# varunagrawal/tiny-faces-pytorch

Measured on AMD Instinct MI355X. Metric: train img/s @ 500x500 bs=12/GPU, higher is better.
Workload: dtype bf16; 1 GPU; configs[2]: bs=12/GPU synthetic 500x500 crops + random boxes; dense_overlap targets on GPU, ResNet-101 hybrid-head fwd, criterion, bwd, fused SGD; global_batch=12, image=500x500, templates=25, parallelism=dp1, weights=random init (tamed kaiming), fp32 master + bf16 MFMA operands

## Files before the change

### tiny-faces-pytorch_amd/csrc/capi.hip

```cpp
#include "common.h"
#include "debug_api.h"

static const char* const kSymbols[] = {
    "tf_version", "tf_build_id", "tf_symbol_count", "tf_symbol_name",
    "tf_targets_workspace_bytes", "tf_dense_overlap_targets", "tf_dense_overlap_iou", "tf_pairwise_iou_distance",
    "tf_nms_workspace_bytes", "tf_nms_f64", "tf_nms_batched_workspace_bytes", "tf_nms_f64_batched",
    "tf_decode_workspace_bytes", "tf_decode_compact",
    "tf_criterion_workspace_bytes", "tf_criterion_fwd_bwd",
    "tf_sgd_step", "tf_image_prepare",
    "tf_conv_mtiles", "tf_conv2d", "tf_pack_weight", "tf_pack_weights_batched", "tf_pack_weights_tiled", "tf_conv2d_wgrad", "tf_conv2d_wgrad_group", "tf_wgrad_workspace_bytes", "tf_unpack_dw",
    "tf_stem_im2col", "tf_stem_conv", "tf_stem_wgrad", "tf_maxpool_fwd", "tf_maxpool_bwd", "tf_maxpool_bwd_stats", "tf_colstats_blocks", "tf_colstats",
    "tf_bn_finalize", "tf_bn_fold", "tf_bn_bwd_finalize", "tf_bn_bwd_apply", "tf_bn_relu", "tf_bn_add_relu",
    "tf_bn_relu_fused", "tf_bn_add_relu_fused", "tf_bn_bwd_apply_fused",
#if TF_EXP
    "tf_conv2d_bnbwd", "tf_conv2d_bnfwd",
#endif
    "tf_upsample_add_crop", "tf_upsample_add_crop_bwd", "tf_reduce_partials",
    "tf_detnet_num_params", "tf_detnet_param_name", "tf_detnet_param_numel", "tf_detnet_workspace_bytes",
    "tf_detnet_out_shape", "tf_detnet_param_region_bytes", "tf_detnet_forward", "tf_detnet_backward", "tf_detnet_ctx_create", "tf_detnet_ctx_destroy", "tf_detnet_forward_ctx", "tf_detnet_backward_ctx", "tf_comm_available", "tf_comm_unique_id", "tf_comm_init", "tf_comm_destroy", "tf_comm_rank", "tf_comm_world", "tf_allreduce_bucket", "tf_comm_join", "tf_comm_allreduce_hook",
    "tf_detnet_set_dual_stream", "tf_detnet_set_grad_events", "tf_detnet_set_grad_callback",
    "tf_detnet_trunk_num_params", "tf_detnet_trunk_param_name", "tf_detnet_trunk_param_numel", "tf_detnet_trunk_workspace_bytes",
    "tf_detnet_trunk_param_region_bytes", "tf_detnet_trunk_forward_ctx", "tf_detnet_trunk_backward_ctx",
    "tf_set_stat_rows", "tf_get_stat_rows", "tf_profile_enable", "tf_profile_collect", "tf_profile_shapes",
};

namespace tf {
static thread_local hipEvent_t g_next_stop_event = nullptr;
void set_next_stop_event(hipEvent_t e) { g_next_stop_event = e; }
hipEvent_t take_next_stop_event() { hipEvent_t e = g_next_stop_event; g_next_stop_event = nullptr; return e; }
}

extern "C" int tf_version(void) { return 610; }
#ifndef TF_BUILD_ID
#define TF_BUILD_ID "unstamped"
#endif
extern "C" const char* tf_build_id(void) { return TF_EXP ? TF_BUILD_ID "+x" : TF_BUILD_ID; }
static int g_stat_rows = 8;
extern "C" int tf_set_stat_rows(int rows) { g_stat_rows = rows <= 0 ? (1 << 30) : (rows > TF_STAT_ROWS ? TF_STAT_ROWS : rows); return TF_OK; }
extern "C" int tf_get_stat_rows(void) { return g_stat_rows; }
extern "C" int tf_symbol_count(void) { return (int)(sizeof(kSymbols) / sizeof(kSymbols[0])); }
extern "C" const char* tf_symbol_name(int i) { return (i >= 0 && i < tf_symbol_count()) ? kSymbols[i] : nullptr; }

namespace {
typedef __bf16 bf16x4 __attribute__((ext_vector_type(4)));
__global__ void probe_tr16_kernel(unsigned short* out) {
  __shared__ __attribute__((aligned(16))) unsigned short lds[256];
  for (int i = threadIdx.x; i < 256; i += 64) lds[i] = (unsigned short)i;
  __syncthreads();
  typedef __attribute__((address_space(3))) bf16x4 lds_bf16x4;
  const bf16x4 v = __builtin_amdgcn_ds_read_tr16_b64_v4bf16((lds_bf16x4*)(lds + threadIdx.x * 4));
  const uint2 raw = __builtin_bit_cast(uint2, v);
  out[threadIdx.x * 4 + 0] = (unsigned short)(raw.x & 0xffff); out[threadIdx.x * 4 + 1] = (unsigned short)(raw.x >> 16);
  out[threadIdx.x * 4 + 2] = (unsigned short)(raw.y & 0xffff); out[threadIdx.x * 4 + 3] = (unsigned short)(raw.y >> 16);
}
}
extern "C" int tf_probe_tr16(unsigned short* out256, void* stream) {
  hipLaunchKernelGGL(probe_tr16_kernel, dim3(1), dim3(64), 0, (hipStream_t)stream, out256);
  TF_CHECK_LAUNCH();
  return TF_OK;
}
```

### tiny-faces-pytorch_amd/csrc/detnet.hip

```cpp
#include <cstdio>
#include <cstdlib>
#include <cstring>
#include <string>
#include <utility>
#include <vector>

#include "common.h"
#include "tuning.h"

extern "C" {
int tf_stem_im2col(const float*, int, int, int, int, void*, int, void*);
int tf_stem_conv(int, const float*, int, int, int, const void*, int, void*, int, const float*, const float*, float*, int*, void*);
int tf_stem_wgrad(int, const float*, int, int, int, const void*, const void*, const float*, const float*, const float*, float*, void*);
int tf_maxpool_fwd(int, const void*, int, int, int, int, const float*, const float*, void*, uint8_t*, void*);
int tf_maxpool_bwd(int, const void*, const uint8_t*, const void*, const float*, const float*, int, int, int, int, void*, void*);
int tf_maxpool_bwd_stats(int, const void*, const uint8_t*, const void*, const float*, const float*, int, int, int, int, void*, float*, int*, void*);
int tf_colstats_blocks(int, int, int);
int tf_colstats(int, const void*, const void*, const void*, const void*, int, int, int, float*, void*);
int tf_bn_finalize(const float*, int, int, int, float, const float*, const float*, float, float, float*, float*, float*, float*, float*,
                   float*, int, void*);
int tf_bn_fold(const float*, const float*, const float*, const float*, float, int, float*, float*, void*);
int tf_bn_bwd_finalize(const float*, int, int, int, int, int, float, const float*, const float*, const float*, float*, float*, float*, float*,
                       float*, int, void*);
int tf_bn_bwd_apply(int, const void*, const void*, const void*, const float*, const float*, const float*, int64_t, int, void*, void*);
// ... 683 lines not shown
extern "C" int tf_detnet_forward(int dtype, int training, const float* x, int N, int H, int W, int nout, void* const* params, float eps,
                                 float mom, float* out, void* ws, size_t ws_bytes, int flags, void* stream_) {
  return tf_detnet_forward_ctx(nullptr, g_force_single ? 1 : 0, dtype, training, x, N, H, W, nout, params, eps, mom, out, ws, ws_bytes, flags, stream_);
}

namespace {

void bn_backward_coefs(Ctx& c, const ConvUnit& u, int C, BnBuf& b, const float* partial, int nblk, int nk, int kidx, int ld, float count,
                       int clear = 1) {
  c.chk(tf_bn_bwd_finalize(partial, nblk, nk, kidx, ld, C, count, c.P(u.gamma), b.mean, b.invstd, c.G(u.gamma), c.G(u.beta), b.cA, b.cB,
                           b.cD, clear, c.stream));
}

tf_wgrad_args wgrad_args(const Ctx& c, const ConvUnit& u, int cout, int N, int H, int W, int OH, int OW, const void* x, int ldx, const void* dy,
                         int lddy, int cin_override = 0, int k_override = 0, int dw_ld = 0) {
  tf_wgrad_args w;
  memset(&w, 0, sizeof(w));
  const int cin = cin_override ? cin_override : u.cin, k = k_override ? k_override : u.k;
  w.dtype = c.dtype; w.N = N; w.H = H; w.W = W; w.Cin = cin; w.OH = OH; w.OW = OW; w.Cout = cout; w.KH = k; w.KW = k;
  w.stride = u.stride; w.pad = u.pad; w.ldx = ldx; w.lddy = lddy; w.x = x; w.dy = dy; w.dw_oihw = c.G(u.w);
  w.dw_ld = dw_ld ? dw_ld : cin * k * k;
  return w;
}

void wgrad(Ctx& c, const ConvUnit& u, int cout, int N, int H, int W, int OH, int OW, const void* x, int ldx, const void* dy, int lddy,
           const BnBuf* pro, int cin_override = 0, int k_override = 0, int dw_ld = 0, float* packed_scratch = nullptr, size_t scratch_floats = 0) {
  const bool skip = tf::tuning().dbg_skip_wgrad;
  if (skip) return;
  const int cin = cin_override ? cin_override : u.cin, k = k_override ? k_override : u.k;
  tf_wgrad_args w = wgrad_args(c, u, cout, N, H, W, OH, OW, x, ldx, dy, lddy, cin_override, k_override, dw_ld);
  if (pro) { w.pro_scale = pro->scale; w.pro_shift = pro->shift; w.pro_relu = 1; }
  if (k > 1 && packed_scratch && c.grads_zeroed) {
    w.partial_ws = packed_scratch; w.partial_ws_bytes = scratch_floats * 4;
    if (tf_wgrad_workspace_bytes(&w) != 0 && tf_wgrad_workspace_bytes(&w) <= w.partial_ws_bytes) {
      const bool w3_off = tf::tuning().wgrad3_off;
      if (!w3_off) { c.chk(tf_conv2d_wgrad(&w, c.wstream())); return; }
    }
    w.partial_ws = nullptr; w.partial_ws_bytes = 0;
  }
  if (k > 1 && packed_scratch) {
    float* oihw = w.dw_oihw;
    w.dw_oihw = packed_scratch; w.packed = 1;
    if (hipMemsetAsync(packed_scratch, 0, (size_t)cout * w.dw_ld * 4, c.wstream()) != hipSuccess) c.chk(TF_ERR_LAUNCH);
    c.chk(tf_conv2d_wgrad(&w, c.wstream()));
    c.chk(tf_unpack_dw(packed_scratch, cout, cin, k * k, oihw, c.wstream()));
    return;
  }
  if (!c.grads_zeroed && hipMemsetAsync(w.dw_oihw, 0, (size_t)cout * w.dw_ld * 4, c.wstream()) != hipSuccess) c.chk(TF_ERR_LAUNCH);
  c.chk(tf_conv2d_wgrad(&w, c.wstream()));
}

}

static std::vector<std::pair<int, hipEvent_t>> g_grad_events;
extern "C" int tf_detnet_set_grad_events(const int* blocks, void* const* events, int n) {
  g_grad_events.clear();
  if (n < 0 || (n > 0 && (!blocks || !events))) return TF_ERR_ARG;
  for (int k = 0; k < n; ++k) g_grad_events.emplace_back(blocks[k], (hipEvent_t)events[k]);
  return TF_OK;
}
static tf_grad_ready_fn g_grad_cb = nullptr;
static void* g_grad_cb_user = nullptr;
extern "C" int tf_detnet_set_grad_callback(tf_grad_ready_fn fn, void* user) { g_grad_cb = fn; g_grad_cb_user = user; return TF_OK; }
static void record_grad_events(const tf_detnet_hooks* h, int block, hipStream_t s, int& rc) {
  if (!h) return;
  bool registered = false;
  for (int k = 0; k < h->n; ++k)
    if (h->blocks[k] == block) {
      registered = true;
      hipEvent_t e = h->events ? (hipEvent_t)h->events[k] : nullptr;
      if (e && hipEventRecord(e, s) != hipSuccess && rc == TF_OK) rc = TF_ERR_LAUNCH;
// ... 325 lines not shown
```

### tiny-faces-pytorch_amd/csrc/wgrad.hip

```cpp
#include "common.h"
#include "tuning.h"
#include "profile.h"

int tf_wgrad_dma_launch(const tf_wgrad_args* a, hipStream_t stream);
int tf_wgrad3x3_launch(const tf_wgrad_args* a, hipStream_t stream);
int tf_wgrad3x3_group_launch(const tf_wgrad_args* a, int n, hipStream_t stream);
int tf_wgrad_pw_group_launch(const tf_wgrad_args* a, int n, hipStream_t stream);

namespace {

typedef __bf16 bf16x8 __attribute__((ext_vector_type(8)));
typedef __bf16 bf16x4 __attribute__((ext_vector_type(4)));
typedef float f32x4 __attribute__((ext_vector_type(4)));

struct WgK {
  const char* x; const char* dy; float* dw;
  const float* pro_scale; const float* pro_shift;
  int H, W, Cin, OH, OW, Cout, KH, KW, stride, pad;
  int M, OHW, ldx, lddy, dw_ld, pro_relu, ci_stride, tap_stride;
  int nco, nci, ntaps, splitk, chunk;
};

template <typename T> struct WgTraits;
template <> struct WgTraits<tf::bf16_t> { static constexpr int PK = 64; };
template <> struct WgTraits<float> { static constexpr int PK = 32; };

__device__ __forceinline__ bf16x8 frag_tr(const char* tile, int pitch, int pk0, int c0) {
  const int l = threadIdx.x & 63, i = l & 15, g = l >> 4;
  const char* p = tile + (pk0 + g * 4 + (i >> 2)) * pitch + (c0 + (i & 3) * 4) * 2;
  typedef __attribute__((address_space(3))) bf16x4 lds_bf16x4;
  const bf16x4 lo = __builtin_amdgcn_ds_read_tr16_b64_v4bf16((lds_bf16x4*)(p));
  const bf16x4 hi = __builtin_amdgcn_ds_read_tr16_b64_v4bf16((lds_bf16x4*)(p + 16 * pitch));
  return __builtin_shufflevector(lo, hi, 0, 1, 2, 3, 4, 5, 6, 7);
}

template <typename T, int BC>
__global__ void __launch_bounds__(256) wgrad_kernel(const WgK a) {
  constexpr int PK = WgTraits<T>::PK;
// ... 141 lines not shown
  k.nco = (A->Cout + BC - 1) / BC; k.nci = (A->Cin + BC - 1) / BC; k.ntaps = A->KH * A->KW;
  const int tiles = k.nco * k.nci * k.ntaps;
  int sk = A->splitk;
  if (sk <= 0) {
    sk = (640 + tiles - 1) / tiles;
    const int maxsk = (k.M + 4 * PK - 1) / (4 * PK);
    if (sk > maxsk) sk = maxsk;
    if (sk < 1) sk = 1;
  }
  k.chunk = (((k.M + sk - 1) / sk) + PK - 1) / PK * PK;
  k.splitk = (k.M + k.chunk - 1) / k.chunk;
  constexpr int PITCH = BC * (int)sizeof(T) + 32;
  const size_t lds = (size_t)4 * PK * PITCH + (A->pro_scale ? (size_t)A->Cin * 8 : 0);
  static tf::PerDevice attr_set;
  if (attr_set.first()) {
    (void)hipFuncSetAttribute(reinterpret_cast<const void*>(&wgrad_kernel<T, BC>), hipFuncAttributeMaxDynamicSharedMemorySize, 160 * 1024);
  }
  const double es = sizeof(T), Md = k.M;
  tf::ProfScope prof(8 + (sizeof(T) == 2 ? 2 : 0) + (BC == 128 ? 1 : 0), 2.0 * Md * A->Cout * A->Cin * k.ntaps,
                     (Md * A->Cout + (double)A->N * A->H * A->W * A->Cin) * es + (double)A->Cout * A->Cin * k.ntaps * 4, stream);
  hipLaunchKernelGGL((wgrad_kernel<T, BC>), dim3(tiles * k.splitk), dim3(256), lds, stream, k);
  return hipGetLastError() == hipSuccess ? TF_OK : TF_ERR_LAUNCH;
}

}

extern "C" int tf_conv2d_wgrad(const tf_wgrad_args* a, void* stream_) {
  hipStream_t stream = (hipStream_t)stream_;
  if (!a || !a->x || !a->dy || !a->dw_oihw) return TF_ERR_ARG;
  if (a->dtype != TF_BF16 && a->dtype != TF_F32) return TF_ERR_UNSUPPORTED;
  const int eps = a->dtype == TF_BF16 ? 8 : 4;
  if (a->ldx % eps || a->lddy % eps || a->ldx < a->Cin || a->lddy < a->Cout) return TF_ERR_ARG;
  if (a->pro_scale && (!a->pro_shift || a->Cin % eps)) return TF_ERR_ARG;
  if ((a->tile == 0 || a->tile == 3) && a->dtype == TF_BF16 && !a->pro_scale) {
    const bool w3_off = tf::tuning().wgrad3_off;
    const int rc = (w3_off && a->tile == 0) ? TF_ERR_UNSUPPORTED : tf_wgrad3x3_launch(a, stream);
    if (rc != TF_ERR_UNSUPPORTED || a->tile == 3) return rc;
  }
  if ((a->tile == 0 || a->tile == 1) && a->dtype == TF_BF16 && !a->pro_scale) return tf_wgrad_dma_launch(a, stream);
  if (a->tile == 1 || a->tile == 3) return TF_ERR_UNSUPPORTED;
  const bool small = a->tile ? a->tile == 64 : true;
  if (a->dtype == TF_BF16) return small ? launch_wgrad<tf::bf16_t, 64>(a, stream) : launch_wgrad<tf::bf16_t, 128>(a, stream);
  return small ? launch_wgrad<float, 64>(a, stream) : launch_wgrad<float, 128>(a, stream);
}

extern "C" int tf_conv2d_wgrad_group(const tf_wgrad_args* probs, int n, void* stream_) {
  hipStream_t stream = (hipStream_t)stream_;
  if (!probs || n <= 0) return TF_ERR_ARG;
  for (int i = 0; i < n; ++i) {
    const tf_wgrad_args& a = probs[i];
    if (!a.x || !a.dy || !a.dw_oihw) return TF_ERR_ARG;
    if (a.dtype != TF_BF16 || a.pro_scale) return TF_ERR_UNSUPPORTED;
    if (a.ldx % 8 || a.lddy % 8 || a.ldx < a.Cin || a.lddy < a.Cout) return TF_ERR_ARG;
    if (a.KH != probs[0].KH || a.KW != probs[0].KW) return TF_ERR_UNSUPPORTED;
  }
  if (probs[0].KH == 1 && probs[0].KW == 1) return tf_wgrad_pw_group_launch(probs, n, stream);
  if (probs[0].KH == 3 && probs[0].KW == 3) return tf_wgrad3x3_group_launch(probs, n, stream);
  return TF_ERR_UNSUPPORTED;
}

namespace {
__global__ void unpack_dw_kernel(const float* __restrict__ p, int Cout, int Cin, int taps, float* __restrict__ out) {
  const size_t total = (size_t)Cout * Cin * taps;
  for (size_t i = (size_t)blockIdx.x * blockDim.x + threadIdx.x; i < total; i += (size_t)gridDim.x * blockDim.x) {
    const int tap = (int)(i % taps);
    const int ci = (int)((i / taps) % Cin);
    const int co = (int)(i / ((size_t)taps * Cin));
    out[i] = p[((size_t)co * taps + tap) * Cin + ci];
  }
}
}
extern "C" int tf_unpack_dw(const float* packed, int Cout, int Cin, int taps, float* dw_oihw, void* stream) {
  if (!packed || !dw_oihw) return TF_ERR_ARG;
// ... 7 lines not shown
```

### tiny-faces-pytorch_amd/csrc/wgrad3x3.hip

```cpp
#include <cstdlib>
#include "common.h"
#include "tuning.h"
#include "profile.h"
#include "lds_dma.h"

namespace {

typedef __bf16 bf16x8 __attribute__((ext_vector_type(8)));
typedef __bf16 bf16x4 __attribute__((ext_vector_type(4)));
typedef float f32x4 __attribute__((ext_vector_type(4)));

__device__ uint4 g_w3zero_page[8];

struct W3K {
  const char* x; const char* dy; float* dw; float* partial;
  int N, H, W, Cin, Cout, ldx, lddy, dw_ld, ci_stride, tap_stride;
  int Hp, Wp, HWp, Mp;
  int nco, nci, splitk, chunk, hb;
  int q64, r64, small_frame, dbg;
  int direct;
};
constexpr int W3_MAXG = 24;
struct W3G { const char* x[W3_MAXG]; const char* dy[W3_MAXG]; float* dw[W3_MAXG]; };

constexpr int PK = 64, NS = 3, YT = PK * 128, XROWS = 512, XBYTES = XROWS * 128, L = 2, NT = 512;
constexpr int TILE_FLOATS = 9 * 64 * 64;

template <int N> __device__ __forceinline__ void wait_vm() { asm volatile("s_waitcnt vmcnt(%0)" ::"n"(N) : "memory"); }
__device__ __forceinline__ void dma16(const void* gsrc, void* lds_wave_base) {
  tf::dma16_hidden(gsrc, tf::lds_addr_uniform(lds_wave_base));
}
__device__ __forceinline__ int fsw(int row) { return ((row >> 1) & 3) << 1; }

typedef __attribute__((address_space(3))) bf16x4 lds_bf16x4;

struct PadPos {
  int n, hp, wp;
  __device__ __forceinline__ void init(int r, const W3K& a) {
    const int kk = (2 * PK + a.HWp - 1) / a.HWp;
    const int rr = r + kk * a.HWp;
    const int q = rr / a.HWp;
    n = q - kk;
    const int rem = rr - q * a.HWp;
    hp = rem / a.Wp; wp = rem - hp * a.Wp;
  }
  template <bool SMALL>
  __device__ __forceinline__ void advance(const W3K& a) {
    wp += a.r64;
    const int c = wp >= a.Wp ? 1 : 0;
    wp -= c * a.Wp;
    hp += a.q64 + c;
    if (SMALL) { while (hp >= a.Hp) { hp -= a.Hp; ++n; } }
    else { const int c2 = hp >= a.Hp ? 1 : 0; hp -= c2 * a.Hp; n += c2; }
  }
  __device__ __forceinline__ bool interior(const W3K& a) const {
    return ((unsigned)n < (unsigned)a.N) & ((unsigned)(hp - 1) < (unsigned)a.H) & ((unsigned)(wp - 1) < (unsigned)a.W);
  }
  __device__ __forceinline__ int pixel(const W3K& a) const { return (n * a.H + (hp - 1)) * a.W + (wp - 1); }
};

typedef float f32x4v __attribute__((ext_vector_type(4)));
constexpr int STG_PITCH = 68;

__device__ __forceinline__ bf16x8 read_tr_pair(const char* base, int off_lo, int off_hi) {
  const bf16x4 lo = __builtin_amdgcn_ds_read_tr16_b64_v4bf16((lds_bf16x4*)(base + off_lo));
  const bf16x4 hi = __builtin_amdgcn_ds_read_tr16_b64_v4bf16((lds_bf16x4*)(base + off_hi));
  return __builtin_shufflevector(lo, hi, 0, 1, 2, 3, 4, 5, 6, 7);
}

template <bool SMALL, bool GROUPED>
__device__ __forceinline__ void wgrad3x3_body(const W3K& a, const char* const gx, const char* const gdy, float* const gdw, int b) {
  extern __shared__ __attribute__((aligned(16))) char smem[];
  char* const yring = smem;
  char* const xring = smem + NS * YT;
  const int ks = b % a.splitk; b /= a.splitk;
  const int tci = b % a.nci; b /= a.nci;
  const int tco = b;
  const int co0 = tco * 64, ci0 = tci * 64;
  const int pb = ks * a.chunk, pe = min(a.Mp, pb + a.chunk);
  const int nst = (pe - pb + PK - 1) / PK;
  const int x0 = pb - PK * a.hb;
  const int D = 2 * a.hb;
  const int tid = threadIdx.x, r = tid >> 3, pslot = tid & 7;
  const int wave_u = __builtin_amdgcn_readfirstlane(tid >> 6);
  const char* zero = reinterpret_cast<const char*>(g_w3zero_page) + pslot * 16;

  const int ls = pslot ^ fsw(r);
  PadPos ypos, xpos;
  ypos.init(pb + r, a);
  xpos.init(x0 + r, a);
  int yrow = pb + r;
  const int ycol = co0 + ls * 8, xcol = ci0 + ls * 8;
  const bool ycok = ycol + 8 <= a.lddy, xcok = xcol + 8 <= a.ldx;
  const char* const ybase = gdy + (size_t)ycol * 2;
  const char* const xbase = gx + (size_t)xcol * 2;
  int ys_slot = 0, xc = 0;
  auto issue_y = [&]() {
    const bool ok = (yrow < pe) & ycok & ypos.interior(a);
    const unsigned off = ok ? (unsigned)ypos.pixel(a) * (unsigned)(a.lddy * 2) : 0u;
    dma16((ok ? ybase : zero) + off, yring + ys_slot * YT + wave_u * 1024);
// ... 47 lines not shown
    if (!(a.dbg & 1)) {
      const char* ys = yring + cs * YT;
      bf16x8 fy0[2], fy1[2], fx0[9], fx1[9];
#pragma unroll
      for (int n = 0; n < 2; ++n) fy0[n] = read_tr_pair(ys, yoff[0][n], yoff[0][n] + 16 * 128);
#pragma unroll
      for (int t = 0; t < 9; ++t) {
        const int o = xoff[t][0];
        fx0[t] = read_tr_pair(xring, o, (o + 16 * 128) & (XBYTES - 1));
        xoff[t][0] = (o + PK * 128) & (XBYTES - 1);
      }
#pragma unroll
      for (int n = 0; n < 2; ++n) fy1[n] = read_tr_pair(ys, yoff[1][n], yoff[1][n] + 16 * 128);
#pragma unroll
      for (int t = 0; t < 9; ++t) {
        const int o = xoff[t][1];
        fx1[t] = read_tr_pair(xring, o, (o + 16 * 128) & (XBYTES - 1));
        xoff[t][1] = (o + PK * 128) & (XBYTES - 1);
      }
      __builtin_amdgcn_sched_barrier(0);
#pragma unroll
      for (int t = 0; t < 9; ++t)
#pragma unroll
        for (int n = 0; n < 2; ++n) acc[t][n] = __builtin_amdgcn_mfma_f32_16x16x32_bf16(fy0[n], fx0[t], acc[t][n], 0, 0, 0);
#pragma unroll
      for (int t = 0; t < 9; ++t)
#pragma unroll
        for (int n = 0; n < 2; ++n) acc[t][n] = __builtin_amdgcn_mfma_f32_16x16x32_bf16(fy1[n], fx1[t], acc[t][n], 0, 0, 0);
    }
    if (++cs == NS) cs = 0;
  }
  wait_vm<0>();

  if (a.partial) {
    if (a.dbg & 2) return;
    float* out = a.partial + ((size_t)ks * (a.nco * a.nci) + (size_t)tco * a.nci + tci) * TILE_FLOATS;
    float* stg = reinterpret_cast<float*>(smem);
#pragma unroll
    for (int t0 = 0; t0 < 9; t0 += 3) {
      __syncthreads();
#pragma unroll
      for (int tl = 0; tl < 3; ++tl)
#pragma unroll
        for (int n = 0; n < 2; ++n)
#pragma unroll
          for (int q = 0; q < 4; ++q)
            stg[(tl * 64 + wco * 32 + n * 16 + lg * 4 + q) * STG_PITCH + wci * 16 + li] = acc[t0 + tl][n][q];
      __syncthreads();
#pragma unroll
      for (int k = 0; k < 6; ++k) {
        const int e4 = tid + k * NT;
        const int row = e4 >> 4, c4 = e4 & 15;
        const f32x4v v = *reinterpret_cast<const f32x4v*>(stg + row * STG_PITCH + c4 * 4);
        *reinterpret_cast<f32x4v*>(out + (size_t)t0 * 4096 + (size_t)e4 * 4) = v;
      }
    }
    return;
  }
#pragma unroll
  for (int t = 0; t < 9; ++t)
#pragma unroll
    for (int n = 0; n < 2; ++n) {
      const int ci = ci0 + wci * 16 + li;
#pragma unroll
      for (int q = 0; q < 4; ++q) {
        const int co = co0 + wco * 32 + n * 16 + lg * 4 + q;
        if (co < a.Cout && ci < a.Cin) {
          float* d = gdw + (size_t)co * a.dw_ld + (size_t)ci * a.ci_stride + (size_t)t * a.tap_stride;
          if (GROUPED || a.direct) *d = acc[t][n][q]; else atomicAdd(d, acc[t][n][q]);
        }
      }
    }
}

template <bool SMALL>
__global__ void __launch_bounds__(NT, 2) wgrad3x3_kernel(const W3K a) {
  wgrad3x3_body<SMALL, false>(a, a.x, a.dy, a.dw, blockIdx.x);
}
template <bool SMALL>
__global__ void __launch_bounds__(NT, 2) wgrad3x3_group_kernel(const W3K a, const W3G g) {
  const int nb = gridDim.x, q = nb >> 3, r = nb & 7, xcd = blockIdx.x & 7, idx = blockIdx.x >> 3;
  const int logical = (xcd < r ? xcd * (q + 1) : r * (q + 1) + (xcd - r) * q) + idx;
  const int per = a.nco * a.nci;
  const int grp = logical / per;
  wgrad3x3_body<SMALL, true>(a, g.x[grp], g.dy[grp], g.dw[grp], logical - grp * per);
}

template <int SG>
__global__ void __launch_bounds__(256) wgrad3x3_reduce_kernel(const W3K a) {
  constexpr int COLS = 256 / SG;
  __shared__ float4 part[SG][COLS + 1];
  const int ntiles = a.nco * a.nci;
  const size_t total4 = (size_t)ntiles * TILE_FLOATS / 4;
  const int col = threadIdx.x % COLS, sg = threadIdx.x / COLS;
  const size_t e4 = (size_t)blockIdx.x * COLS + col;
  const size_t stride = (size_t)ntiles * TILE_FLOATS;
  float4 s = make_float4(0.f, 0.f, 0.f, 0.f);
  if (e4 < total4) {
    const float* src = a.partial + e4 * 4;
#pragma unroll 4
    for (int ks = sg; ks < a.splitk; ks += SG) {
      const float4 v = *reinterpret_cast<const float4*>(src + (size_t)ks * stride);
      s.x += v.x; s.y += v.y; s.z += v.z; s.w += v.w;
    }
  }
  if (SG > 1) {
    part[sg][col] = s;
    __syncthreads();
    if (sg != 0) return;
#pragma unroll
    for (int g = 1; g < SG; ++g) { const float4 v = part[g][col]; s.x += v.x; s.y += v.y; s.z += v.z; s.w += v.w; }
  }
  if (e4 >= total4) return;
  const size_t e = e4 * 4;
  const int tile = (int)(e / TILE_FLOATS), rem = (int)(e - (size_t)tile * TILE_FLOATS);
  const int t = rem / 4096, co = (tile / a.nci) * 64 + (rem % 4096) / 64, ci = (tile % a.nci) * 64 + rem % 64;
  if (co >= a.Cout) return;
  float* d = a.dw + (size_t)co * a.dw_ld + (size_t)t * a.tap_stride;
  const float v[4] = {s.x, s.y, s.z, s.w};
#pragma unroll
  for (int j = 0; j < 4; ++j)
    if (ci + j < a.Cin) d[(size_t)(ci + j) * a.ci_stride] += v[j];
}

bool w3_plan(const tf_wgrad_args* A, W3K& k) {
  if (A->dtype != TF_BF16 || A->pro_scale) return false;
  if (A->KH != 3 || A->KW != 3 || A->stride != 1 || A->pad != 1 || A->OH != A->H || A->OW != A->W) return false;
  if (A->W + 3 > 2 * PK) return false;
  k.x = (const char*)A->x; k.dy = (const char*)A->dy; k.dw = A->dw_oihw; k.partial = nullptr;
  k.N = A->N; k.H = A->H; k.W = A->W; k.Cin = A->Cin; k.Cout = A->Cout; k.ldx = A->ldx; k.lddy = A->lddy; k.dw_ld = A->dw_ld;
  if (A->packed) { k.ci_stride = 1; k.tap_stride = A->Cin; } else { k.ci_stride = 9; k.tap_stride = 1; }
  k.Hp = A->H + 2; k.Wp = A->W + 2; k.HWp = k.Hp * k.Wp;
  const long long mp = (long long)A->N * k.HWp;
  if (mp > (1ll << 30)) return false;
  if ((long long)A->N * A->H * A->W * 2 * (A->ldx > A->lddy ? A->ldx : A->lddy) >= (1ll << 32)) return false;
  k.Mp = (int)mp;
  k.hb = (k.Wp + 1 + PK - 1) / PK;
  k.q64 = PK / k.Wp; k.r64 = PK % k.Wp; k.small_frame = k.Hp <= k.q64 + 1; k.dbg = 0; k.direct = 0;
  k.nco = (A->Cout + 63) / 64; k.nci = (A->Cin + 63) / 64;
  const int tiles = k.nco * k.nci;
  int sk = A->splitk;
  if (sk <= 0) {
    const int target = tf::tuning().wgrad3_blocks;
    sk = (target + tiles - 1) / tiles;
    const int maxsk = (k.Mp + 6 * PK - 1) / (6 * PK);
    if (sk > maxsk) sk = maxsk;
    if (sk < 1) sk = 1;
  }
  k.chunk = (((k.Mp + sk - 1) / sk) + PK - 1) / PK * PK;
  k.splitk = (k.Mp + k.chunk - 1) / k.chunk;
  return true;
}

}

extern "C" size_t tf_wgrad_workspace_bytes(const tf_wgrad_args* A) {
  W3K k;
  if (!A || !w3_plan(A, k)) return 0;
  return (size_t)k.splitk * k.nco * k.nci * TILE_FLOATS * sizeof(float);
}

int tf_wgrad3x3_launch(const tf_wgrad_args* A, hipStream_t stream) {
  W3K k;
  if (!w3_plan(A, k)) return TF_ERR_UNSUPPORTED;
  const size_t need = (size_t)k.splitk * k.nco * k.nci * TILE_FLOATS * sizeof(float);
  const bool atomics_only = tf::tuning().wgrad3_atomics;
  if (A->partial_ws && A->partial_ws_bytes >= need && !atomics_only) k.partial = (float*)A->partial_ws;
  const int dbg = tf::tuning().wgrad3_dbg;
  k.dbg = dbg;
  const size_t lds = (size_t)NS * YT + XBYTES;
  static tf::PerDevice attr_set;
  if (attr_set.first()) {
    (void)hipFuncSetAttribute(reinterpret_cast<const void*>(&wgrad3x3_kernel<false>), hipFuncAttributeMaxDynamicSharedMemorySize, 160 * 1024);
    (void)hipFuncSetAttribute(reinterpret_cast<const void*>(&wgrad3x3_kernel<true>), hipFuncAttributeMaxDynamicSharedMemorySize, 160 * 1024);
  }
  const double Md = (double)A->N * A->H * A->W;
  tf::ProfScope prof(16, 2.0 * Md * A->Cout * A->Cin * 9, (Md * A->Cout + Md * A->Cin) * 2 + (double)A->Cout * A->Cin * 9 * 4, stream, (int)Md,
                     A->Cout, A->Cin * 9, 9, 2, 0);
  if (k.small_frame) hipLaunchKernelGGL(wgrad3x3_kernel<true>, dim3(k.nco * k.nci * k.splitk), dim3(NT), lds, stream, k);
  else hipLaunchKernelGGL(wgrad3x3_kernel<false>, dim3(k.nco * k.nci * k.splitk), dim3(NT), lds, stream, k);
  if (k.partial) {
    const size_t total4 = (size_t)k.nco * k.nci * TILE_FLOATS / 4;
    if (k.splitk >= 128)     hipLaunchKernelGGL(wgrad3x3_reduce_kernel<16>, dim3((unsigned)(total4 / 16)), dim3(256), 0, stream, k);
    else if (k.splitk >= 32) hipLaunchKernelGGL(wgrad3x3_reduce_kernel<4>, dim3((unsigned)(total4 / 64)), dim3(256), 0, stream, k);
    else if (k.splitk >= 16) hipLaunchKernelGGL(wgrad3x3_reduce_kernel<2>, dim3((unsigned)(total4 / 128)), dim3(256), 0, stream, k);
    else                     hipLaunchKernelGGL(wgrad3x3_reduce_kernel<1>, dim3((unsigned)(total4 / 256)), dim3(256), 0, stream, k);
  }
  return hipGetLastError() == hipSuccess ? TF_OK : TF_ERR_LAUNCH;
}

int tf_wgrad3x3_group_launch(const tf_wgrad_args* A, int n, hipStream_t stream) {
  if (n <= 0 || n > W3_MAXG) return TF_ERR_UNSUPPORTED;
  tf_wgrad_args first = A[0];
  first.splitk = 1; first.partial_ws = nullptr; first.partial_ws_bytes = 0;
  W3K k;
  if (!w3_plan(&first, k) || k.splitk != 1) return TF_ERR_UNSUPPORTED;
  W3G g;
  for (int i = 0; i < n; ++i) {
    const tf_wgrad_args& q = A[i];
    if (q.dtype != first.dtype || q.pro_scale || q.N != first.N || q.H != first.H || q.W != first.W || q.Cin != first.Cin || q.Cout != first.Cout ||
        q.KH != 3 || q.KW != 3 || q.stride != 1 || q.pad != 1 || q.OH != q.H || q.OW != q.W || q.ldx != first.ldx || q.lddy != first.lddy ||
        q.dw_ld != first.dw_ld || q.packed != first.packed) return TF_ERR_UNSUPPORTED;
    g.x[i] = (const char*)q.x; g.dy[i] = (const char*)q.dy; g.dw[i] = q.dw_oihw;
  }
  for (int i = n; i < W3_MAXG; ++i) { g.x[i] = nullptr; g.dy[i] = nullptr; g.dw[i] = nullptr; }
  k.direct = 1;
  const size_t lds = (size_t)NS * YT + XBYTES;
  static tf::PerDevice attr_set;
  if (attr_set.first()) {
    (void)hipFuncSetAttribute(reinterpret_cast<const void*>(&wgrad3x3_group_kernel<false>), hipFuncAttributeMaxDynamicSharedMemorySize, 160 * 1024);
    (void)hipFuncSetAttribute(reinterpret_cast<const void*>(&wgrad3x3_group_kernel<true>), hipFuncAttributeMaxDynamicSharedMemorySize, 160 * 1024);
  }
  const double Md = (double)first.N * first.H * first.W;
  tf::ProfScope prof(19, 2.0 * Md * first.Cout * first.Cin * 9 * n, ((Md * first.Cout + Md * first.Cin) * 2 + (double)first.Cout * first.Cin * 9 * 4) * n, stream,
                     (int)Md, first.Cout, first.Cin * 9, 9, 2, 0, -1.0, true);
  const dim3 grid(k.nco * k.nci * n);
  if (k.small_frame) TF_LAUNCH_TIMED((wgrad3x3_group_kernel<true>), grid, dim3(NT), lds, stream, k, g);
  else TF_LAUNCH_TIMED((wgrad3x3_group_kernel<false>), grid, dim3(NT), lds, stream, k, g);
  return hipGetLastError() == hipSuccess ? TF_OK : TF_ERR_LAUNCH;
}
// ... 1 lines not shown
```

Before: 1356 img/s.

## Add dedicated stride-2 3x3 wgrad kernel with polyphase LDS staging

Adds a new MFMA weight-gradient kernel for 3x3 stride-2 convolutions. It splits the input into four polyphase planes streamed into an LDS ring via DMA, so each tap reads contiguous rows. It reuses the existing split-K partial workspace and reduce path, and factors the store, split and reduce logic into shared helpers. Stride-2 units in the detnet backward now request tile 4, moving them off the generic DMA or templated wgrad path. This adds new kernel complexity and a dependency on workspace size.

Result: no change. 1364 img/s (median of 6 runs) (+0.6%).

```diff
diff --git a/tiny-faces-pytorch_amd/csrc/capi.hip b/tiny-faces-pytorch_amd/csrc/capi.hip
--- a/tiny-faces-pytorch_amd/csrc/capi.hip
+++ b/tiny-faces-pytorch_amd/csrc/capi.hip
@@ -30,7 +30,7 @@
 hipEvent_t take_next_stop_event() { hipEvent_t e = g_next_stop_event; g_next_stop_event = nullptr; return e; }
 }
 
-extern "C" int tf_version(void) { return 610; }
+extern "C" int tf_version(void) { return 611; }
 #ifndef TF_BUILD_ID
 #define TF_BUILD_ID "unstamped"
 #endif
diff --git a/tiny-faces-pytorch_amd/csrc/detnet.hip b/tiny-faces-pytorch_amd/csrc/detnet.hip
--- a/tiny-faces-pytorch_amd/csrc/detnet.hip
+++ b/tiny-faces-pytorch_amd/csrc/detnet.hip
@@ -739,11 +739,13 @@
   if (pro) { w.pro_scale = pro->scale; w.pro_shift = pro->shift; w.pro_relu = 1; }
   if (k > 1 && packed_scratch && c.grads_zeroed) {
     w.partial_ws = packed_scratch; w.partial_ws_bytes = scratch_floats * 4;
-    if (tf_wgrad_workspace_bytes(&w) != 0 && tf_wgrad_workspace_bytes(&w) <= w.partial_ws_bytes) {
+    if (u.stride == 2) w.tile = 4;
+    const size_t need = tf_wgrad_workspace_bytes(&w);
+    if (need != 0 && need <= w.partial_ws_bytes) {
       const bool w3_off = tf::tuning().wgrad3_off;
       if (!w3_off) { c.chk(tf_conv2d_wgrad(&w, c.wstream())); return; }
     }
-    w.partial_ws = nullptr; w.partial_ws_bytes = 0;
+    w.partial_ws = nullptr; w.partial_ws_bytes = 0; w.tile = 0;
   }
   if (k > 1 && packed_scratch) {
     float* oihw = w.dw_oihw;
diff --git a/tiny-faces-pytorch_amd/csrc/wgrad.hip b/tiny-faces-pytorch_amd/csrc/wgrad.hip
--- a/tiny-faces-pytorch_amd/csrc/wgrad.hip
+++ b/tiny-faces-pytorch_amd/csrc/wgrad.hip
@@ -4,6 +4,7 @@
 
 int tf_wgrad_dma_launch(const tf_wgrad_args* a, hipStream_t stream);
 int tf_wgrad3x3_launch(const tf_wgrad_args* a, hipStream_t stream);
+int tf_wgrad3x3s2_launch(const tf_wgrad_args* a, hipStream_t stream);
 int tf_wgrad3x3_group_launch(const tf_wgrad_args* a, int n, hipStream_t stream);
 int tf_wgrad_pw_group_launch(const tf_wgrad_args* a, int n, hipStream_t stream);
 
@@ -211,13 +212,21 @@
   const int eps = a->dtype == TF_BF16 ? 8 : 4;
   if (a->ldx % eps || a->lddy % eps || a->ldx < a->Cin || a->lddy < a->Cout) return TF_ERR_ARG;
   if (a->pro_scale && (!a->pro_shift || a->Cin % eps)) return TF_ERR_ARG;
-  if ((a->tile == 0 || a->tile == 3) && a->dtype == TF_BF16 && !a->pro_scale) {
-    const bool w3_off = tf::tuning().wgrad3_off;
-    const int rc = (w3_off && a->tile == 0) ? TF_ERR_UNSUPPORTED : tf_wgrad3x3_launch(a, stream);
-    if (rc != TF_ERR_UNSUPPORTED || a->tile == 3) return rc;
+  if ((a->tile == 0 || a->tile == 3 || a->tile == 4) && a->dtype == TF_BF16 && !a->pro_scale) {
+    const bool w3_off = tf::tuning().wgrad3_off && a->tile == 0;
+    if (a->tile != 4) {
+      const int rc = w3_off ? TF_ERR_UNSUPPORTED : tf_wgrad3x3_launch(a, stream);
+      if (rc != TF_ERR_UNSUPPORTED || a->tile == 3) return rc;
+    }
+    tf_wgrad_args q = *a;
+    q.tile = 4;
+    const size_t ws = a->partial_ws ? tf_wgrad_workspace_bytes(&q) : 0;
+    const bool s2 = a->tile == 4 || (!w3_off && ws != 0 && a->partial_ws_bytes >= ws);
+    const int rc = s2 ? tf_wgrad3x3s2_launch(a, stream) : TF_ERR_UNSUPPORTED;
+    if (rc != TF_ERR_UNSUPPORTED || a->tile == 4) return rc;
   }
   if ((a->tile == 0 || a->tile == 1) && a->dtype == TF_BF16 && !a->pro_scale) return tf_wgrad_dma_launch(a, stream);
-  if (a->tile == 1 || a->tile == 3) return TF_ERR_UNSUPPORTED;
+  if (a->tile == 1 || a->tile == 3 || a->tile == 4) return TF_ERR_UNSUPPORTED;
   const bool small = a->tile ? a->tile == 64 : true;
   if (a->dtype == TF_BF16) return small ? launch_wgrad<tf::bf16_t, 64>(a, stream) : launch_wgrad<tf::bf16_t, 128>(a, stream);
   return small ? launch_wgrad<float, 64>(a, stream) : launch_wgrad<float, 128>(a, stream);
diff --git a/tiny-faces-pytorch_amd/csrc/wgrad3x3.hip b/tiny-faces-pytorch_amd/csrc/wgrad3x3.hip
--- a/tiny-faces-pytorch_amd/csrc/wgrad3x3.hip
+++ b/tiny-faces-pytorch_amd/csrc/wgrad3x3.hip
@@ -19,6 +19,7 @@
   int nco, nci, splitk, chunk, hb;
   int q64, r64, small_frame, dbg;
   int direct;
+  int OH, OW, deep;
 };
 constexpr int W3_MAXG = 24;
 struct W3G { const char* x[W3_MAXG]; const char* dy[W3_MAXG]; float* dw[W3_MAXG]; };
@@ -66,6 +67,52 @@
   const bf16x4 lo = __builtin_amdgcn_ds_read_tr16_b64_v4bf16((lds_bf16x4*)(base + off_lo));
   const bf16x4 hi = __builtin_amdgcn_ds_read_tr16_b64_v4bf16((lds_bf16x4*)(base + off_hi));
   return __builtin_shufflevector(lo, hi, 0, 1, 2, 3, 4, 5, 6, 7);
+}
+
+template <bool GROUPED>
+__device__ __forceinline__ void w3_store(const W3K& a, const f32x4 (&acc)[9][2], int ks, int tco, int tci, float* const gdw, char* smem, int tid) {
+  const int co0 = tco * 64, ci0 = tci * 64;
+  const int wave = tid >> 6, wco = wave & 1, wci = wave >> 1;
+  const int l = tid & 63, li = l & 15, lg = l >> 4;
+  if (a.partial) {
+    if (a.dbg & 2) return;
+    float* out = a.partial + ((size_t)ks * (a.nco * a.nci) + (size_t)tco * a.nci + tci) * TILE_FLOATS;
+    float* stg = reinterpret_cast<float*>(smem);
+#pragma unroll
+    for (int t0 = 0; t0 < 9; t0 += 3) {
+      __syncthreads();
+#pragma unroll
+      for (int tl = 0; tl < 3; ++tl)
+#pragma unroll
+        for (int n = 0; n < 2; ++n)
+#pragma unroll
+          for (int q = 0; q < 4; ++q)
+            stg[(tl * 64 + wco * 32 + n * 16 + lg * 4 + q) * STG_PITCH + wci * 16 + li] = acc[t0 + tl][n][q];
+      __syncthreads();
+#pragma unroll
+      for (int k = 0; k < 6; ++k) {
+        const int e4 = tid + k * NT;
+        const int row = e4 >> 4, c4 = e4 & 15;
+        const f32x4v v = *reinterpret_cast<const f32x4v*>(stg + row * STG_PITCH + c4 * 4);
+        *reinterpret_cast<f32x4v*>(out + (size_t)t0 * 4096 + (size_t)e4 * 4) = v;
+      }
+    }
+    return;
+  }
+#pragma unroll
+  for (int t = 0; t < 9; ++t)
+#pragma unroll
+    for (int n = 0; n < 2; ++n) {
+      const int ci = ci0 + wci * 16 + li;
+#pragma unroll
+      for (int q = 0; q < 4; ++q) {
+        const int co = co0 + wco * 32 + n * 16 + lg * 4 + q;
+        if (co < a.Cout && ci < a.Cin) {
+          float* d = gdw + (size_t)co * a.dw_ld + (size_t)ci * a.ci_stride + (size_t)t * a.tap_stride;
+          if (GROUPED || a.direct) *d = acc[t][n][q]; else atomicAdd(d, acc[t][n][q]);
+        }
+      }
+    }
 }
 
 template <bool SMALL, bool GROUPED>
@@ -179,45 +226,7 @@
   }
   wait_vm<0>();
 
-  if (a.partial) {
-    if (a.dbg & 2) return;
-    float* out = a.partial + ((size_t)ks * (a.nco * a.nci) + (size_t)tco * a.nci + tci) * TILE_FLOATS;
-    float* stg = reinterpret_cast<float*>(smem);
-#pragma unroll
-    for (int t0 = 0; t0 < 9; t0 += 3) {
-      __syncthreads();
-#pragma unroll
-      for (int tl = 0; tl < 3; ++tl)
-#pragma unroll
-        for (int n = 0; n < 2; ++n)
-#pragma unroll
-          for (int q = 0; q < 4; ++q)
-            stg[(tl * 64 + wco * 32 + n * 16 + lg * 4 + q) * STG_PITCH + wci * 16 + li] = acc[t0 + tl][n][q];
-      __syncthreads();
-#pragma unroll
-      for (int k = 0; k < 6; ++k) {
-        const int e4 = tid + k * NT;
-        const int row = e4 >> 4, c4 = e4 & 15;
-        const f32x4v v = *reinterpret_cast<const f32x4v*>(stg + row * STG_PITCH + c4 * 4);
-        *reinterpret_cast<f32x4v*>(out + (size_t)t0 * 4096 + (size_t)e4 * 4) = v;
-      }
-    }
-    return;
-  }
-#pragma unroll
-  for (int t = 0; t < 9; ++t)
-#pragma unroll
-    for (int n = 0; n < 2; ++n) {
-      const int ci = ci0 + wci * 16 + li;
-#pragma unroll
-      for (int q = 0; q < 4; ++q) {
-        const int co = co0 + wco * 32 + n * 16 + lg * 4 + q;
-        if (co < a.Cout && ci < a.Cin) {
-          float* d = gdw + (size_t)co * a.dw_ld + (size_t)ci * a.ci_stride + (size_t)t * a.tap_stride;
-          if (GROUPED || a.direct) *d = acc[t][n][q]; else atomicAdd(d, acc[t][n][q]);
-        }
-      }
-    }
+  w3_store<GROUPED>(a, acc, ks, tco, tci, gdw, smem, tid);
 }
 
 template <bool SMALL>
@@ -231,6 +240,132 @@
   const int per = a.nco * a.nci;
   const int grp = logical / per;
   wgrad3x3_body<SMALL, true>(a, g.x[grp], g.dy[grp], g.dw[grp], logical - grp * per);
+}
+
+constexpr int S2_PLANE = 4 * PK * 128;
+constexpr int S2_X = 4 * S2_PLANE;
+constexpr size_t S2_LDS = (size_t)S2_X + NS * YT;
+
+template <bool SMALL>
+__global__ void __launch_bounds__(NT, 2) wgrad3x3_s2_kernel(const W3K a) {
+  extern __shared__ __attribute__((aligned(16))) char smem[];
+  char* const xring = smem;
+  char* const yring = smem + S2_X;
+  int b = blockIdx.x;
+  const int ks = b % a.splitk; b /= a.splitk;
+  const int tci = b % a.nci; b /= a.nci;
+  const int tco = b;
+  const int co0 = tco * 64, ci0 = tci * 64;
+  const int pb = ks * a.chunk, pe = min(a.Mp, pb + a.chunk);
+  const int nst = (pe - pb + PK - 1) / PK;
+  const int tid = threadIdx.x, r = tid >> 3, pslot = tid & 7;
+  const int wave_u = __builtin_amdgcn_readfirstlane(tid >> 6);
+  const char* zero = reinterpret_cast<const char*>(g_w3zero_page) + pslot * 16;
+  const int ls = pslot ^ fsw(r);
+  PadPos ypos, xpos;
+  ypos.init(pb + r, a);
+  xpos.init(pb + r, a);
+  int yrow = pb + r;
+  const int ycol = co0 + ls * 8, xcol = ci0 + ls * 8;
+  const bool ycok = ycol + 8 <= a.lddy, xcok = xcol + 8 <= a.ldx;
+  const char* const ybase = a.dy + (size_t)ycol * 2;
+  const char* const xbase = a.x + (size_t)xcol * 2;
+  const unsigned xrs = (unsigned)(a.ldx * 2), xrow = (unsigned)a.W * xrs;
+  int ys_slot = 0, xc = 0;
+  auto issue_y = [&]() {
+    const bool ok = (yrow < pe) & ycok & ((unsigned)ypos.n < (unsigned)a.N) & (ypos.hp < a.OH) & (ypos.wp < a.OW);
+    const unsigned off = ok ? (unsigned)((ypos.n * a.OH + ypos.hp) * a.OW + ypos.wp) * (unsigned)(a.lddy * 2) : 0u;
+    dma16((ok ? ybase : zero) + off, yring + ys_slot * YT + wave_u * 1024);
+    ypos.template advance<SMALL>(a); yrow += PK;
+    if (++ys_slot == NS) ys_slot = 0;
+  };
+  auto issue_x = [&]() {
+    const int ih = 2 * xpos.hp - 1, iw = 2 * xpos.wp - 1;
+    const bool nok = xcok & ((unsigned)xpos.n < (unsigned)a.N);
+    const bool r0 = (unsigned)ih < (unsigned)a.H, r1 = (unsigned)(ih + 1) < (unsigned)a.H;
+    const bool c0 = (unsigned)iw < (unsigned)a.W, c1 = (unsigned)(iw + 1) < (unsigned)a.W;
+    const unsigned o00 = (unsigned)((xpos.n * a.H + ih) * a.W + iw) * xrs, o01 = o00 + xrs, o10 = o00 + xrow, o11 = o10 + xrs;
+    char* const dst = xring + (xc & 3) * (PK * 128) + wave_u * 1024;
+    const bool k00 = nok & r0 & c0, k01 = nok & r0 & c1, k10 = nok & r1 & c0, k11 = nok & r1 & c1;
+    dma16((k00 ? xbase : zero) + (k00 ? o00 : 0u), dst);
+    dma16((k01 ? xbase : zero) + (k01 ? o01 : 0u), dst + S2_PLANE);
+    dma16((k10 ? xbase : zero) + (k10 ? o10 : 0u), dst + 2 * S2_PLANE);
+    dma16((k11 ? xbase : zero) + (k11 ? o11 : 0u), dst + 3 * S2_PLANE);
+    xpos.template advance<SMALL>(a);
+    ++xc;
+  };
+
+  f32x4 acc[9][2];
+#pragma unroll
+  for (int t = 0; t < 9; ++t)
+#pragma unroll
+    for (int n = 0; n < 2; ++n) acc[t][n] = f32x4{0.f, 0.f, 0.f, 0.f};
+  const int wave = tid >> 6, wco = wave & 1, wci = wave >> 1;
+  const int l = tid & 63, li = l & 15, lg = l >> 4;
+  const int frow = lg * 4 + (li >> 2), fhalf = (li & 1) << 3, fs = (li & 3) >> 1;
+  int yoff[2][2];
+#pragma unroll
+  for (int k = 0; k < 2; ++k)
+#pragma unroll
+    for (int n = 0; n < 2; ++n) {
+      const int row = k * 32 + frow, slot = ((wco * 32 + n * 16) >> 3) + fs;
+      yoff[k][n] = row * 128 + ((slot ^ fsw(row)) << 4) + fhalf;
+    }
+  int xoff[9][2];
+#pragma unroll
+  for (int t = 0; t < 9; ++t)
+#pragma unroll
+    for (int k = 0; k < 2; ++k) {
+      const int shift = (t / 3 >> 1) * a.Wp + (t % 3 >> 1);
+      const int row = (k * 32 + shift + frow) & (4 * PK - 1);
+      const int slot = ((wci * 16) >> 3) + fs;
+      xoff[t][k] = row * 128 + ((slot ^ fsw(row)) << 4) + fhalf;
+    }
+
+  for (int c = 0; c < 3; ++c) issue_x();
+  issue_y(); issue_y();
+  int cs = 0;
+  for (int st = 0; st < nst; ++st) {
+    if (st == 0) wait_vm<1>();
+    else if (a.deep) wait_vm<3>();
+    else wait_vm<5>();
+    __builtin_amdgcn_s_barrier();
+    issue_x(); issue_y();
+    if (!(a.dbg & 1)) {
+      const char* ys = yring + cs * YT;
+      bf16x8 fy0[2], fy1[2], fx0[9], fx1[9];
+#pragma unroll
+      for (int n = 0; n < 2; ++n) fy0[n] = read_tr_pair(ys, yoff[0][n], yoff[0][n] + 16 * 128);
+#pragma unroll
+      for (int t = 0; t < 9; ++t) {
+        const char* xp = xring + ((t / 3 & 1) * 2 + (t % 3 & 1)) * S2_PLANE;
+        const int o = xoff[t][0];
+        fx0[t] = read_tr_pair(xp, o, (o + 16 * 128) & (S2_PLANE - 1));
+        xoff[t][0] = (o + PK * 128) & (S2_PLANE - 1);
+      }
+#pragma unroll
+      for (int n = 0; n < 2; ++n) fy1[n] = read_tr_pair(ys, yoff[1][n], yoff[1][n] + 16 * 128);
+#pragma unroll
+      for (int t = 0; t < 9; ++t) {
+        const char* xp = xring + ((t / 3 & 1) * 2 + (t % 3 & 1)) * S2_PLANE;
+        const int o = xoff[t][1];
+        fx1[t] = read_tr_pair(xp, o, (o + 16 * 128) & (S2_PLANE - 1));
+        xoff[t][1] = (o + PK * 128) & (S2_PLANE - 1);
+      }
+      __builtin_amdgcn_sched_barrier(0);
+#pragma unroll
+      for (int t = 0; t < 9; ++t)
+#pragma unroll
+        for (int n = 0; n < 2; ++n) acc[t][n] = __builtin_amdgcn_mfma_f32_16x16x32_bf16(fy0[n], fx0[t], acc[t][n], 0, 0, 0);
+#pragma unroll
+      for (int t = 0; t < 9; ++t)
+#pragma unroll
+        for (int n = 0; n < 2; ++n) acc[t][n] = __builtin_amdgcn_mfma_f32_16x16x32_bf16(fy1[n], fx1[t], acc[t][n], 0, 0, 0);
+    }
+    if (++cs == NS) cs = 0;
+  }
+  wait_vm<0>();
+  w3_store<false>(a, acc, ks, tco, tci, a.dw, smem, tid);
 }
 
 template <int SG>
@@ -270,6 +405,21 @@
     if (ci + j < a.Cin) d[(size_t)(ci + j) * a.ci_stride] += v[j];
 }
 
+void w3_split(const tf_wgrad_args* A, W3K& k) {
+  k.nco = (A->Cout + 63) / 64; k.nci = (A->Cin + 63) / 64;
+  const int tiles = k.nco * k.nci;
+  int sk = A->splitk;
+  if (sk <= 0) {
+    const int target = tf::tuning().wgrad3_blocks;
+    sk = (target + tiles - 1) / tiles;
+    const int maxsk = (k.Mp + 6 * PK - 1) / (6 * PK);
+    if (sk > maxsk) sk = maxsk;
+    if (sk < 1) sk = 1;
+  }
+  k.chunk = (((k.Mp + sk - 1) / sk) + PK - 1) / PK * PK;
+  k.splitk = (k.Mp + k.chunk - 1) / k.chunk;
+}
+
 bool w3_plan(const tf_wgrad_args* A, W3K& k) {
   if (A->dtype != TF_BF16 || A->pro_scale) return false;
   if (A->KH != 3 || A->KW != 3 || A->stride != 1 || A->pad != 1 || A->OH != A->H || A->OW != A->W) return false;
@@ -284,26 +434,45 @@
   k.Mp = (int)mp;
   k.hb = (k.Wp + 1 + PK - 1) / PK;
   k.q64 = PK / k.Wp; k.r64 = PK % k.Wp; k.small_frame = k.Hp <= k.q64 + 1; k.dbg = 0; k.direct = 0;
-  k.nco = (A->Cout + 63) / 64; k.nci = (A->Cin + 63) / 64;
-  const int tiles = k.nco * k.nci;
-  int sk = A->splitk;
-  if (sk <= 0) {
-    const int target = tf::tuning().wgrad3_blocks;
-    sk = (target + tiles - 1) / tiles;
-    const int maxsk = (k.Mp + 6 * PK - 1) / (6 * PK);
-    if (sk > maxsk) sk = maxsk;
-    if (sk < 1) sk = 1;
-  }
-  k.chunk = (((k.Mp + sk - 1) / sk) + PK - 1) / PK * PK;
-  k.splitk = (k.Mp + k.chunk - 1) / k.chunk;
+  k.OH = A->OH; k.OW = A->OW; k.deep = 0;
+  w3_split(A, k);
   return true;
+}
+
+bool w3s2_plan(const tf_wgrad_args* A, W3K& k) {
+  if (A->dtype != TF_BF16 || A->pro_scale) return false;
+  if (A->KH != 3 || A->KW != 3 || A->stride != 2 || A->pad != 1 || A->H < 1 || A->W < 1) return false;
+  if (A->OH != (A->H - 1) / 2 + 1 || A->OW != (A->W - 1) / 2 + 1 || A->OW + 1 > 2 * PK - 1) return false;
+  k.x = (const char*)A->x; k.dy = (const char*)A->dy; k.dw = A->dw_oihw; k.partial = nullptr;
+  k.N = A->N; k.H = A->H; k.W = A->W; k.Cin = A->Cin; k.Cout = A->Cout; k.ldx = A->ldx; k.lddy = A->lddy; k.dw_ld = A->dw_ld;
+  if (A->packed) { k.ci_stride = 1; k.tap_stride = A->Cin; } else { k.ci_stride = 9; k.tap_stride = 1; }
+  k.OH = A->OH; k.OW = A->OW;
+  k.Hp = A->OH + 1; k.Wp = A->OW + 1; k.HWp = k.Hp * k.Wp;
+  const long long mp = (long long)A->N * k.HWp;
+  if (mp > (1ll << 30)) return false;
+  if ((long long)A->N * A->H * A->W * 2 * A->ldx >= (1ll << 32)) return false;
+  if ((long long)A->N * A->OH * A->OW * 2 * A->lddy >= (1ll << 32)) return false;
+  k.Mp = (int)mp;
+  k.hb = 0;
+  k.q64 = PK / k.Wp; k.r64 = PK % k.Wp; k.small_frame = k.Hp <= k.q64 + 1; k.dbg = 0; k.direct = 0;
+  k.deep = (PK - 1) + (k.Wp + 1) >= 2 * PK;
+  w3_split(A, k);
+  return true;
+}
+
+void w3_reduce(const W3K& k, hipStream_t stream) {
+  const size_t total4 = (size_t)k.nco * k.nci * TILE_FLOATS / 4;
+  if (k.splitk >= 128)     hipLaunchKernelGGL(wgrad3x3_reduce_kernel<16>, dim3((unsigned)(total4 / 16)), dim3(256), 0, stream, k);
+  else if (k.splitk >= 32) hipLaunchKernelGGL(wgrad3x3_reduce_kernel<4>, dim3((unsigned)(total4 / 64)), dim3(256), 0, stream, k);
+  else if (k.splitk >= 16) hipLaunchKernelGGL(wgrad3x3_reduce_kernel<2>, dim3((unsigned)(total4 / 128)), dim3(256), 0, stream, k);
+  else                     hipLaunchKernelGGL(wgrad3x3_reduce_kernel<1>, dim3((unsigned)(total4 / 256)), dim3(256), 0, stream, k);
 }
 
 }
 
 extern "C" size_t tf_wgrad_workspace_bytes(const tf_wgrad_args* A) {
   W3K k;
-  if (!A || !w3_plan(A, k)) return 0;
+  if (!A || !(w3_plan(A, k) || (A->tile == 4 && w3s2_plan(A, k)))) return 0;
   return (size_t)k.splitk * k.nco * k.nci * TILE_FLOATS * sizeof(float);
 }
 
@@ -326,13 +495,27 @@
                      A->Cout, A->Cin * 9, 9, 2, 0);
   if (k.small_frame) hipLaunchKernelGGL(wgrad3x3_kernel<true>, dim3(k.nco * k.nci * k.splitk), dim3(NT), lds, stream, k);
   else hipLaunchKernelGGL(wgrad3x3_kernel<false>, dim3(k.nco * k.nci * k.splitk), dim3(NT), lds, stream, k);
-  if (k.partial) {
-    const size_t total4 = (size_t)k.nco * k.nci * TILE_FLOATS / 4;
-    if (k.splitk >= 128)     hipLaunchKernelGGL(wgrad3x3_reduce_kernel<16>, dim3((unsigned)(total4 / 16)), dim3(256), 0, stream, k);
-    else if (k.splitk >= 32) hipLaunchKernelGGL(wgrad3x3_reduce_kernel<4>, dim3((unsigned)(total4 / 64)), dim3(256), 0, stream, k);
-    else if (k.splitk >= 16) hipLaunchKernelGGL(wgrad3x3_reduce_kernel<2>, dim3((unsigned)(total4 / 128)), dim3(256), 0, stream, k);
-    else                     hipLaunchKernelGGL(wgrad3x3_reduce_kernel<1>, dim3((unsigned)(total4 / 256)), dim3(256), 0, stream, k);
-  }
+  if (k.partial) w3_reduce(k, stream);
+  return hipGetLastError() == hipSuccess ? TF_OK : TF_ERR_LAUNCH;
+}
+
+int tf_wgrad3x3s2_launch(const tf_wgrad_args* A, hipStream_t stream) {
+  W3K k;
+  if (!w3s2_plan(A, k)) return TF_ERR_UNSUPPORTED;
+  const size_t need = (size_t)k.splitk * k.nco * k.nci * TILE_FLOATS * sizeof(float);
+  if (A->partial_ws && A->partial_ws_bytes >= need && !tf::tuning().wgrad3_atomics) k.partial = (float*)A->partial_ws;
+  k.dbg = tf::tuning().wgrad3_dbg;
+  static tf::PerDevice attr_set;
+  if (attr_set.first()) {
+    (void)hipFuncSetAttribute(reinterpret_cast<const void*>(&wgrad3x3_s2_kernel<false>), hipFuncAttributeMaxDynamicSharedMemorySize, 160 * 1024);
+    (void)hipFuncSetAttribute(reinterpret_cast<const void*>(&wgrad3x3_s2_kernel<true>), hipFuncAttributeMaxDynamicSharedMemorySize, 160 * 1024);
+  }
+  const double Md = (double)A->N * A->OH * A->OW;
+  tf::ProfScope prof(16, 2.0 * Md * A->Cout * A->Cin * 9, (Md * A->Cout + (double)A->N * A->H * A->W * A->Cin) * 2 + (double)A->Cout * A->Cin * 9 * 4,
+                     stream, (int)Md, A->Cout, A->Cin * 9, 9, 2, 0, 2.0 * k.Mp * A->Cout * A->Cin * 9);
+  if (k.small_frame) hipLaunchKernelGGL(wgrad3x3_s2_kernel<true>, dim3(k.nco * k.nci * k.splitk), dim3(NT), S2_LDS, stream, k);
+  else hipLaunchKernelGGL(wgrad3x3_s2_kernel<false>, dim3(k.nco * k.nci * k.splitk), dim3(NT), S2_LDS, stream, k);
+  if (k.partial) w3_reduce(k, stream);
   return hipGetLastError() == hipSuccess ? TF_OK : TF_ERR_LAUNCH;
 }
 
```
